# CoderWZW/ARLib

Measured on AMD Instinct MI355X. Metric: BPR-train interactions/sec (LightGCN d=64 L=3 + BPR + Adam, B=2048), higher is better.
Workload: dtype f32

## Files before the change

### arlib_amd/_lib.py

```python
import ctypes as C
import os

_HERE = os.path.dirname(os.path.abspath(__file__))
LIB_PATH = os.environ.get('ARLIB_AMD_LIB') or os.path.join(_HERE, 'lib', 'libarlib_amd.so')
ABI_VERSION = 27
_lib = None


class ArlError(RuntimeError):
    pass


class arl_csr(C.Structure):
    _fields_ = [('n_rows', C.c_int64), ('nnz', C.c_int64), ('rowptr', C.c_void_p), ('col', C.c_void_p), ('val', C.c_void_p),
                ('chunk', C.c_int32), ('n_chunks', C.c_int64), ('chunk_row', C.c_void_p), ('chunk_begin', C.c_void_p),
                ('chunk_end', C.c_void_p), ('n_long', C.c_int64), ('long_row', C.c_void_p), ('long_first', C.c_void_p),
                ('long_count', C.c_void_p), ('partial', C.c_void_p), ('row_tasks', C.c_void_p)]


class arl_blocked(C.Structure):
    _fields_ = [('n_waves', C.c_int64), ('rows_per_wave', C.c_int64), ('loads_in_flight', C.c_int64), ('wave_ptr', C.c_void_p), ('wave_rows', C.c_void_p), ('rec_col', C.c_void_p),
                ('rec_val', C.c_void_p), ('n_split', C.c_int64), ('split_row', C.c_void_p), ('split_first', C.c_void_p), ('split_count', C.c_void_p),
                ('partial', C.c_void_p), ('waves_per_group', C.c_int64)]


class arl_tiled(C.Structure):
    _fields_ = [('n_sweeps', C.c_int64), ('n_slots', C.c_int64), ('cap', C.c_int64), ('n_cb', C.c_int64), ('nnz', C.c_int64),
                ('n_groups', C.c_int64), ('bin_rows', C.c_void_p), ('seg_ptr', C.c_void_p), ('e_col', C.c_void_p), ('e_val', C.c_void_p),
                ('e_row', C.c_void_p)]


_vp, _i64, _i32, _f = C.c_void_p, C.c_int64, C.c_int32, C.c_float
_SIGS = {
    'arl_abi_version': (C.c_int, []),
    'arl_mt_seed': (C.c_int, [_vp, _vp, _i64]),
    'arl_sampler_shuffle': (C.c_int, [_vp, _vp, _i64]),
    'arl_mt_sample_range': (C.c_int, [_vp, _i64, _i64, C.c_int32, _vp, _vp]),
    'arl_sampler_next_batch': (C.c_int, [_vp, _vp, _i64, _i64, _i32, _vp, _vp, _i64, _vp, _vp, _vp]),
    'arl_norm_adj_values_f32': (C.c_int, [_i64, _vp, _vp, _vp, _vp, _vp, _vp]),
    'arl_norm_adj_values_coo_f32': (C.c_int, [_i64, _vp, _vp, _vp, _vp, _i64, _vp, _vp, _vp]),
    'arl_norm_vals_coo_f32': (C.c_int, [_vp, _vp, _vp, _i64, _vp, _vp, _vp]),
    'arl_spmm_csr_f32': (C.c_int, [C.POINTER(arl_csr), _vp, _i64, _f, _f, _vp, _vp, _vp]),
    'arl_spmm_csr_layersum_f32': (C.c_int, [C.POINTER(arl_csr), _vp, _i64, _vp, _vp, _vp, _vp]),
    'arl_spmm_csr_adam_f32': (C.c_int, [C.POINTER(arl_csr), _vp, _i64, _f, _f, _vp, _vp, _vp, _vp, _vp, _f, _f, _f, _f, _i64, _vp]),
    'arl_spmm_blocked_f32': (C.c_int, [C.POINTER(arl_blocked), _vp, _i64, _f, _f, _vp, _vp, _vp, _vp]),
    'arl_spmm_csr_rscale_f32': (C.c_int, [C.POINTER(arl_csr), _vp, _i64, _vp, _f, _f, _vp, _vp, _vp]),
    'arl_spmm_blocked_rscale_f32': (C.c_int, [C.POINTER(arl_blocked), _vp, _i64, _vp, _f, _f, _vp, _vp, _vp]),
    'arl_spmm_blocked_layersum_f32': (C.c_int, [C.POINTER(arl_blocked), _vp, _i64, _vp, _vp, _vp, _vp]),
    'arl_spmm_blocked_adam_f32': (C.c_int, [C.POINTER(arl_blocked), _vp, _i64, _f, _f, _vp, _vp, _vp, _vp, _vp, _f, _f, _f, _f, _i64, _vp]),
    'arl_lpt_deal': (C.c_int, [_i64, _vp, _i64, _i64, _vp, _vp]),
    'arl_syn_v1_pairs': (_i64, [_i64, _i64, C.c_double, C.c_uint64, C.c_double, _i64, _i64, _vp, _i64]),
    'arl_graph_digest': (C.c_uint64, [_vp, _i64]),
    'arl_spmm_tiled_f32': (C.c_int, [C.POINTER(arl_tiled), _vp, _i64, _f, _f, _vp, _vp, _vp, _vp]),
    'arl_spmm_tiled_adam_f32': (C.c_int, [C.POINTER(arl_tiled), _vp, _i64, _f, _f, _vp, _vp, _vp, _vp, _vp, _f, _f, _f, _f, _i64, _vp]),
    'arl_spmm_csr_flagged_f32': (C.c_int, [C.POINTER(arl_csr), _vp, _i64, _vp, _f, _f, _vp, _vp, _vp, _vp]),
    'arl_spmm_csr_rows_workspace_bytes': (_i64, [_i64, _i64, _i64]),
    'arl_spmm_csr_rows_f32': (C.c_int, [C.POINTER(arl_csr), _vp, _i64, _vp, _i64, _i64, _vp, _i64, _f, _vp, _vp, _vp, _vp]),
    'arl_mark_rows_u8': (C.c_int, [_vp, _vp, _i64, _i32, _vp]),
    'arl_mark_rows_bits_u32': (C.c_int, [_vp, _vp, _i64, _i32, _vp]),
    'arl_zero_rows_f32': (C.c_int, [_vp, _vp, _i64, _i64, _vp]),
    'arl_batch_rows_set_f32': (C.c_int, [_vp, _vp, _vp, _vp, _i64, _i64, _vp, _f, _vp, _vp, _vp]),
    'arl_batch_rows_clear_f32': (C.c_int, [_vp, _vp, _vp, _vp, _i64, _i64, _vp, _vp]),
    'arl_bpr_l2_workspace_bytes': (_i64, [_i64]),
    'arl_bpr_l2_fwd_bwd_f32': (C.c_int, [_vp, _i64, _i64, _vp, _vp, _vp, _i64, _f, _f, _vp, _vp, _vp, _i32, _vp]),
    'arl_bpr_l2_partial_f32': (C.c_int, [_vp, _i64, _i64, _vp, _vp, _vp, _i64, _i64, _vp, _vp, _vp]),
    'arl_bpr_l2_backward_f32': (C.c_int, [_vp, _i64, _i64, _vp, _vp, _vp, _i64, _f, _f, _vp, _vp, _vp, _vp]),
    'arl_adam_dense_f32': (C.c_int, [_vp, _vp, _vp, _vp, _i64, _f, _f, _f, _f, _i64, _vp]),
    'arl_sgd_dense_f32': (C.c_int, [_vp, _vp, _i64, _f, _vp]),
    'arl_gather_rows_f32': (C.c_int, [_vp, _vp, _i64, _i64, _vp, _vp]),
    'arl_scatter_add_rows_f32': (C.c_int, [_vp, _vp, _i64, _i64, _vp, _f, _vp]),
    'arl_rows_axpy_unique_f32': (C.c_int, [_vp, _vp, _vp, _i64, _i64, _f, _vp, _vp]),
    'arl_shard_batch_prep_i32': (C.c_int, [_vp, _vp, _vp, _i64, _i64, _i64, _vp, _vp, _vp, _vp, _vp]),
    'arl_infonce_workspace_bytes': (_i64, [_i64, _i64]),
    'arl_infonce_fwd_bwd_f32': (C.c_int, [_vp, _vp, _i64, _i64, _f, _f, _vp, _vp, _vp, _vp, _vp]),
    'arl_simgcl_perturb_f32': (C.c_int, [_vp, _vp, _i64, _i64, _f, _vp]),
    'arl_simgcl_perturb_rng_f32': (C.c_int, [_vp, _vp, _i64, _i64, _vp, _f, C.c_uint64, C.c_uint64, _vp]),
    'arl_ngcf_combine_f32': (C.c_int, [_vp, _vp, _i64, _i64, _vp, _vp]),
    'arl_ngcf_act_f32': (C.c_int, [_vp, _vp, _i64, _i64, _f, _vp]),
    'arl_ngcf_act_bwd_f32': (C.c_int, [_vp, _vp, _i64, _i64, _f, _vp, _vp]),
    'arl_ngcf_combine_bwd_f32': (C.c_int, [_vp, _vp, _vp, _i64, _i64, _vp, _vp, _vp]),
    'arl_ngcf_dense_fwd_f32': (C.c_int, [_vp, _vp, _vp, _i64, _i64, _f, _vp, _vp]),
    'arl_ngcf_dense_dgrad_f32': (C.c_int, [_vp, _vp, _vp, _vp, _vp, _i64, _i64, _f, _vp, _vp, _vp, _vp]),
    'arl_ngcf_wgrad_workspace_bytes': (_i64, [_i64, _i64]),
    'arl_ngcf_dense_wgrad_f32': (C.c_int, [_vp, _vp, _vp, _i64, _i64, _vp, _vp, _vp]),
    'arl_ncf_tower_fwd_f32': (C.c_int, [_vp, _vp, _vp, _i64, _i64, _vp, _vp, _vp, _vp, _vp, _vp, _vp, _vp, _vp, _vp]),
    'arl_ncf_tower_bwd_workspace_bytes': (_i64, [_i64, _i64]),
    'arl_ncf_tower_bwd_f32': (C.c_int, [_vp, _vp, _vp, _vp, _vp, _vp, _i64, _i64, _vp, _vp, _vp, _vp, _vp, _vp, _vp]),
    'arl_wrmf_l2_workspace_bytes': (_i64, [_i64]),
# ... 74 lines not shown
```

### arlib_amd/csrc/arl_host.cpp

```cpp
#include <cstdint>
#include <cstddef>
#include <queue>
#include <cmath>
#include <algorithm>
#include <utility>
#include <vector>
#include "arlib_amd.h"

namespace {

class PyMersenne {
public:
    explicit PyMersenne(uint32_t *state) : w_(state), pos_(state[kN]) {}
    ~PyMersenne() { w_[kN] = pos_; }

    uint32_t next32() {
        if (pos_ >= kN) refill();
        uint32_t y = w_[pos_++];
        y ^= y >> 11;
        y ^= (y << 7) & 0x9d2c5680u;
        y ^= (y << 15) & 0xefc60000u;
        return y ^ (y >> 18);
    }

// ... 23 lines not shown
        w[kN] = kN;
    }

private:
    static constexpr uint32_t kN = 624, kM = 397;
    static uint32_t twist(uint32_t hi, uint32_t lo, uint32_t far) {
        const uint32_t y = (hi & 0x80000000u) | (lo & 0x7fffffffu);
        return far ^ (y >> 1) ^ ((y & 1u) ? 0x9908b0dfu : 0u);
    }
    void refill() {
        for (uint32_t k = 0; k < kN - kM; ++k) w_[k] = twist(w_[k], w_[k + 1], w_[k + kM]);
        for (uint32_t k = kN - kM; k < kN - 1; ++k) w_[k] = twist(w_[k], w_[k + 1], w_[k + kM - kN]);
        w_[kN - 1] = twist(w_[kN - 1], w_[0], w_[kM - 1]);
        pos_ = 0;
    }
    uint32_t *w_;
    uint32_t pos_;
};

inline bool user_has_item(const int64_t *rowptr, const int32_t *items, int64_t rows, int32_t user, int32_t item) {
    if (user < 0 || user >= rows) return false;
    const int32_t *lo = items + rowptr[user], *hi = items + rowptr[user + 1];
    while (lo < hi) {
        const int32_t *mid = lo + (hi - lo) / 2;
        if (*mid < item) lo = mid + 1; else hi = mid;
    }
    return lo < items + rowptr[user + 1] && *lo == item;
}

}

extern "C" {

int arl_abi_version(void) { return 27; }

int arl_mt_seed(uint32_t *mt_state, const uint32_t *key, int64_t key_len) {
    if (!mt_state || !key) return ARL_E_NULL;
    if (key_len < 1) return ARL_E_ARG;
    PyMersenne::seed_by_array(mt_state, key, key_len);
    return ARL_OK;
}

int arl_sampler_shuffle(uint32_t *mt_state, int32_t *pairs, int64_t nnz) {
    if (!mt_state || (!pairs && nnz > 0)) return ARL_E_NULL;
    if (nnz < 0 || nnz > 0xFFFFFFFFll) return ARL_E_RANGE;
    if (mt_state[624] > 624) return ARL_E_ARG;
    PyMersenne rng(mt_state);
    int64_t *rows = reinterpret_cast<int64_t *>(pairs);
    const bool aligned = (reinterpret_cast<uintptr_t>(pairs) & 7u) == 0;
    constexpr int kAhead = 512;
    int64_t js[kAhead];
    for (int64_t i = nnz - 1; i >= 1;) {
        const int cnt = (int)(i < kAhead ? i : kAhead);
        for (int t = 0; t < cnt; ++t) {
            js[t] = rng.below((uint32_t)(i - t + 1));
            __builtin_prefetch(pairs + 2 * js[t], 1, 0);
        }
        if (aligned) {
            for (int t = 0; t < cnt; ++t) { const int64_t a = i - t, j = js[t], v = rows[a]; rows[a] = rows[j]; rows[j] = v; }
        } else {
            for (int t = 0; t < cnt; ++t)
                for (int c = 0; c < 2; ++c) { const int64_t a = i - t, j = js[t]; const int32_t v = pairs[2 * a + c]; pairs[2 * a + c] = pairs[2 * j + c]; pairs[2 * j + c] = v; }
        }
        i -= cnt;
    }
    return ARL_OK;
}
// ... 130 lines not shown
```

### arlib_amd/csrc/arl_kernels.hip

```cpp
#include <hip/hip_runtime.h>
#include <stdint.h>
#include <math.h>
#include <stdio.h>
#include <stdlib.h>
#include "arlib_amd.h"
#include <type_traits>

#define ARL_LAUNCH_CHECK()                                  \
    do {                                                    \
        hipError_t e__ = hipGetLastError();                 \
        if (e__ != hipSuccess) return (int)e__;             \
    } while (0)

namespace {

constexpr int kWave = 64;
constexpr int kBlock = 256;
constexpr int kWavesPerBlock = kBlock / kWave;

__device__ __forceinline__ float wave_sum(float v) {
#pragma unroll
    for (int off = 32; off > 0; off >>= 1) v += __shfl_xor(v, off);
    return v;
}
// ... 417 lines not shown
#pragma unroll
                    for (int i = 0; i < 4; ++i) { const int k = k0 + 64 * i + lane; x[q][i] = k < d ? s[k] : 0.f; }
                }
#pragma unroll
                for (int q = 0; q < 4; ++q) {
                    if (tt[q] < 0) continue;
#pragma unroll
                    for (int i = 0; i < 4; ++i) { const float c = sc[q] * x[q][i]; acc[i] = acc[i] + c; }
                }
            }
        });
        if (!owner) return;
#pragma unroll
        for (int i = 0; i < 4; ++i) { const int k = k0 + 64 * i + lane; if (k < d) o[k] = acc[i]; }
    }
    if (MARK && lane == 0) {
        flags[row] = 1;
        atomicOr(bits + (row >> 5), 1u << (row & 31));
    }
}
__global__ __launch_bounds__(kBlock) void batch_rows_clear_kernel(float *__restrict__ G, uint8_t *__restrict__ flags, uint32_t *__restrict__ bits,
                                                                   const int32_t *__restrict__ idx, int n, int d, uint32_t *__restrict__ dup) {
    const int lane = threadIdx.x & 63;
    const int t = blockIdx.x * kWavesPerBlock + (threadIdx.x >> 6);
    if (t >= n) return;
    const int row = idx[t];
    float *o = G + (size_t)row * d;
    for (int k = lane; k < d; k += kWave) o[k] = 0.f;
    if (lane == 0) {
        flags[row] = 0;
        atomicAnd(bits + (row >> 5), ~(1u << (row & 31)));
        if (dup) atomicAnd(dup + (row >> 5), ~(1u << (row & 31)));
    }
}

struct TiledDev {
    int n_sweeps, n_slots, cap, n_cb, n_groups;
    const int32_t *bin_rows;
    const int32_t *seg_ptr;
    const int32_t *e_col;
    const float *e_val;
    const uint16_t *e_row;
};

constexpr int kTiledThreads = 1024;
constexpr int kTiledWaves = kTiledThreads / kWave;

template <int LPR, int MODE>
__global__ __launch_bounds__(kTiledThreads) void spmm_tiled_kernel(TiledDev T, const float *__restrict__ X, int d, Epi ep) {
    constexpr int G = kWave / LPR;
    extern __shared__ float acc_lds[];
    const int ld = d + 4;
    const int tid = threadIdx.x, lane = tid & 63, wv = tid >> 6;
    const int g = lane / LPR, q = lane % LPR;
    const int og = wv * G + g;
    const bool qact = q * 4 < d;
    const float *xq = X + q * 4;
    for (int sweep = 0; sweep < T.n_sweeps; ++sweep) {
        const int bin = sweep * T.n_slots + blockIdx.x;
        for (int t = tid; t < T.cap * ld; t += kTiledThreads) acc_lds[t] = 0.f;
        const int lo = T.seg_ptr[(size_t)bin * T.n_groups + og], hi = T.seg_ptr[(size_t)bin * T.n_groups + og + 1];
        __syncthreads();
        int c_n = 0, r_n = -1;
        float v_n = 0.f;
        if (lo + q < hi) { c_n = T.e_col[lo + q]; v_n = T.e_val[lo + q]; r_n = T.e_row[lo + q]; }
        for (int base = lo; __any(base < hi); base += LPR) {
// ... 3619 lines not shown

int arl_spmm_tiled_f32(const arl_tiled *T, const float *X, int64_t d, float alpha, float beta, const float *Z, const uint8_t *zflags, float *Y,
                       arl_stream_t stream) {
    if (!Y) return ARL_E_NULL;
    if (beta != 0.f && !Z) return ARL_E_NULL;
    if (Y == X) return ARL_E_ARG;
    Epi ep = {};
    ep.alpha = alpha; ep.beta = beta; ep.Z = (beta != 0.f) ? Z : nullptr; ep.zflags = zflags; ep.Y = Y;
    return launch_spmm_tiled<EPI_AXPBY>(T, X, d, ep, (hipStream_t)stream);
}

int arl_spmm_tiled_adam_f32(const arl_tiled *T, const float *X, int64_t d, float alpha, float beta, const float *Z, const uint8_t *zflags,
                            float *P, float *M, float *V, float lr, float beta1, float beta2, float eps, int64_t step, arl_stream_t stream) {
    if (!P || !M || !V) return ARL_E_NULL;
    if (beta != 0.f && !Z) return ARL_E_NULL;
    if (step < 1 || P == X) return ARL_E_ARG;
    Epi ep = {};
    ep.alpha = alpha; ep.beta = beta; ep.Z = (beta != 0.f) ? Z : nullptr; ep.zflags = zflags; ep.P = P; ep.M = M; ep.V = V;
    {
        const AdamScalars a = adam_scalars(lr, beta1, beta2, step);
        ep.step_size = a.step_size; ep.bc2_sqrt = a.bc2_sqrt; ep.w1 = a.w1; ep.b2 = a.b2; ep.w2 = a.w2; ep.eps = (float)typed_double(eps);
    }
    return launch_spmm_tiled<EPI_ADAM>(T, X, d, ep, (hipStream_t)stream);
}

int arl_spmm_csr_flagged_f32(const arl_csr *A, const float *X, int64_t d, const uint32_t *xbits, float alpha, float beta, const float *Z,
                             const uint8_t *zflags, float *Y, arl_stream_t stream) {
    if (!Y) return ARL_E_NULL;
    if (beta != 0.f && !Z) return ARL_E_NULL;
    if (Y == X) return ARL_E_ARG;
    Epi ep = {};
    ep.alpha = alpha; ep.beta = beta; ep.Z = (beta != 0.f) ? Z : nullptr; ep.zflags = zflags; ep.Y = Y;
    return launch_spmm<EPI_AXPBY>(A, X, d, ep, (hipStream_t)stream, xbits);
}

int arl_spmm_csr_adam_f32(const arl_csr *A, const float *X, int64_t d, float alpha, float beta, const float *Z, const uint8_t *zflags, float *P,
                          float *M, float *V, float lr, float beta1, float beta2, float eps, int64_t step, arl_stream_t stream) {
    if (!P || !M || !V) return ARL_E_NULL;
    if (beta != 0.f && !Z) return ARL_E_NULL;
    if (step < 1) return ARL_E_ARG;
    if (P == X) return ARL_E_ARG;
    Epi ep = {};
    ep.alpha = alpha; ep.beta = beta; ep.Z = (beta != 0.f) ? Z : nullptr; ep.zflags = zflags; ep.P = P; ep.M = M; ep.V = V;
    {
        const AdamScalars a = adam_scalars(lr, beta1, beta2, step);
        ep.step_size = a.step_size; ep.bc2_sqrt = a.bc2_sqrt; ep.w1 = a.w1; ep.b2 = a.b2; ep.w2 = a.w2; ep.eps = (float)typed_double(eps);
    }
    return launch_spmm<EPI_ADAM>(A, X, d, ep, (hipStream_t)stream);
}

int64_t arl_spmm_csr_rows_workspace_bytes(int64_t n_rows_sel, int64_t nsplit, int64_t d) {
    return (n_rows_sel < 0 || nsplit < 1 || d < 0) ? 0 : (int64_t)sizeof(float) * n_rows_sel * nsplit * d;
}

int arl_spmm_csr_rows_f32(const arl_csr *A, const float *X, int64_t d, const int32_t *rows, int64_t n_rows_sel, int64_t nsplit,
                          const float *const *layers, int64_t n_layers, float alpha, const float *row_weight, float *out_c, void *workspace,
                          arl_stream_t stream) {
    if (!A || !X || !rows || !out_c || !workspace || !A->rowptr) return ARL_E_NULL;
    if (A->nnz > 0 && (!A->col || !A->val)) return ARL_E_NULL;
    if (n_layers < 0 || n_layers > 8 || (n_layers > 0 && !layers)) return ARL_E_ARG;
    if (d <= 0 || d > 256 || (d & 3)) return ARL_E_DIM;
    if (n_rows_sel < 0 || nsplit < 1 || nsplit > 1024 || n_rows_sel * nsplit > 0x7fffffffll) return ARL_E_RANGE;
    if (n_rows_sel == 0) return ARL_OK;
    hipStream_t st = (hipStream_t)stream;
    CsrDev D = {};
    D.n_rows = (int)A->n_rows; D.rowptr = A->rowptr; D.col = A->col; D.val = A->val;
// ... 1086 lines not shown
```

### arlib_amd/engine.py

```python
import torch

from . import ops


def mean_adjacency_gradient(A, E0, G, L, s, out, noises=None, eps=0.1):
    if L == 0:
        return out
    E = [E0]
    for k in range(L - 1):
        nxt = ops.spmm(A, E[-1])
        if noises is not None:
            ops.simgcl_perturb_(nxt, noises[k], eps)
        E.append(nxt)
    G = G.contiguous()
    acc = G
    for j in range(L):
        ops.sddmm_csr(A, acc, E[L - 1 - j], s, out=out)
        if j < L - 1:
            acc = ops.spmm(A, acc, 1.0, 1.0, G)
    return out


class PropagationEngine:
    def __init__(self, graph, n_users, n_items, emb_size, n_layers, reg, lr, device, skip_layer0=False,
# ... 6 lines not shown
        self.optimizer = optimizer
        self.device = torch.device(device)
        if self.device.type != 'cuda':
            raise ops._lib.ArlError('PropagationEngine needs a GPU device (no CPU fallback)')
        if graph is None and self.L > 0:
            raise ValueError('n_layers > 0 needs a graph')
        if graph is not None and graph.n_rows != self.N:
            raise ValueError('graph has %d rows, expected U+I=%d' % (graph.n_rows, self.N))
        if self.L > 0:
            ops._check_width(self.d, 'PropagationEngine')
        if self.skip0 and self.L < 1:
            raise ValueError('skip_layer0 needs n_layers >= 1')
        if schedule not in ('auto', 'csr', 'blocked'):
            raise ValueError("schedule must be 'auto', 'csr' or 'blocked'")
        if schedule != 'csr':
            ops.auto_blocked(graph, emb_size, split=self.U, force=(schedule == 'blocked'))
        if graph is not None and graph.nnz >= ops.BLOCKED_MIN_NNZ:
            graph.enable_masked_order()
        z = lambda: torch.zeros(self.N, self.d, dtype=torch.float32, device=self.device)
        self.E0 = z() if table is None else table
        if self.E0.shape != (self.N, self.d) or self.E0.dtype != torch.float32 or not self.E0.is_contiguous():
            raise ValueError('table must be contiguous fp32 [U+I, d]')
        self.m, self.v, self.G = z(), z(), z()
        if self.L > 0:
            self.S, self.Ea, self.Eb = z(), z(), z()
        else:
            self.S = self.E0
        self.t = 0
        self.loss_out = torch.zeros(4, dtype=torch.float32, device=self.device)
        self._G_dirty = True
        self._noise_seed, self._noise_stream = None, 0
        self.nsplit = 32
        self.flags = self.bits = self.dup_bits = self.hops = None
        self._sparse_B, self._sb_cache = None, {}
        self.Gc = self.out_c = self.rows_ws = self.ar = self.arB = self._ws = None
        self._sgl_acc = self._sgl_hops = None
        self.ngcf_W = self.ngcf_m = self.ngcf_v = None

    @property
    def user_emb(self):
        return self.E0[:self.U]

    @property
    def item_emb(self):
        return self.E0[self.U:]

    def forward(self, noises=None, eps=0.1, out=None):
        L, A = self.L, self.A
        if L == 0:
            return self.E0
        S = self.S if out is None else out
        if noises is None and not self.skip0:
            if L == 1:
                return ops.spmm(A, self.E0, 0.5, 0.5, self.E0, out=S)
            ops.spmm_layersum(A, self.E0, self.E0, S, self.Ea)
            cur, nxt = self.Ea, self.Eb
            for _ in range(L - 2):
                ops.spmm_layersum(A, cur, S, S, nxt)
                cur, nxt = nxt, cur
            s = 1.0 / (L + 1)
            return ops.spmm(A, cur, s, s, S, out=S)
        cur, nxt, x = self.Ea, self.Eb, self.E0
        for k in range(L):
            ops.spmm(A, x, out=cur)
            if noises is not None:
                ops.simgcl_perturb_(cur, noises[k], eps)
# ... 51 lines not shown
    def _begin_sparse(self, B):
        self._sparse_buffers(B)
        if self._G_dirty:
            self.G.zero_()
            self._G_dirty = False

    def _batch_rows(self, u, p, n):
        return torch.cat([u, p + self.U, n + self.U])

    def _contrast_rows(self, u, p):
        uidx = torch.unique(u.long())
        iidx = torch.unique(p.long()) + self.U
        return torch.cat([uidx, iidx]).to(torch.int32), uidx.numel()

    def _streams(self, n):
        if self._noise_seed is None:
            self._noise_seed = int(torch.randint(0, 2 ** 62, (1,)).item())
            self._noise_stream = 0
        first = self._noise_stream
        self._noise_stream += n
        return self._noise_seed, first

    def _mean_rows(self, graph, hops, rows, out=None, workspace=None):
        layers = [self.E0]
        for k in range(self.L - 1):
            layers.append(ops.spmm(graph, layers[-1], out=hops[k]))
        return ops.spmm_rows(graph, layers[-1], rows, layers, 1.0 / (self.L + 1), nsplit=self.nsplit, out=out, workspace=workspace, check_range=False)

    def _bpr_compact(self, out_c, B):
        self.Gc.zero_()
        ops.bpr_l2_fwd_bwd(out_c, B, self.ar, self.ar, self.arB, self.reg, self.Gc, workspace=self._ws, loss_out=self.loss_out, check_range=False, distinct_rows=True)

    def _set_rows(self, rows, grad):
        ops.batch_rows_set_(self.G, self.flags, self.bits, rows, grad, 1.0, check_range=False, dup_bits=self.dup_bits)

    def _mark_rows(self, rows):
        ops.mark_rows_(self.flags, rows, 1, check_range=False)
        ops.mark_bits_(self.bits, rows, True, self.N, check_range=False)

    def _clear_rows(self, rows):
        ops.batch_rows_clear_(self.G, self.flags, self.bits, rows, check_range=False, dup_bits=self.dup_bits)

    def _masked_hops(self, graph, bufs, src=None, after_hop=None):
        acc, bits = self.G if src is None else src, self.bits
        for k in range(self.L - 1):
            acc = ops.spmm_flagged(graph, acc, bits, 1.0, 1.0, self.G, self.flags, out=bufs[k % len(bufs)])
            bits = None
            if after_hop is not None:
                after_hop(self.L - 1 - k, acc)
        return acc, bits

    def loss_and_grad_out(self, out, u, p, n):
        self.G.zero_()
        self._G_dirty = True
        if self._ws is None or self._ws.numel() < 4 * u.numel():
            self._ws = torch.empty(4 * u.numel(), dtype=torch.float32, device=self.device)
        ops.bpr_l2_fwd_bwd(out, self.U, u, p, n, self.reg, self.G, workspace=self._ws, loss_out=self.loss_out, check_range=False)
        return self.loss_out

    def grad(self, u, p, n):
        out = self.forward()
        lo = self.loss_and_grad_out(out, u, p, n)
        return lo, self.backward_to_table(self.G)

    def step(self, u, p, n, rows=None):
        if self.optimizer != 'adam' or self.L == 0 or self.skip0 or self.L > 8:
            return self.step_dense(u, p, n)
        return self._step_sparse(u, p, n, rows, None)

    def _step_sparse(self, u, p, n, rows, extra_grad):
        L, A = self.L, self.A
        B = u.numel()
        if rows is None:
            rows = self._batch_rows(u, p, n)
        self._begin_sparse(B)
        s = 1.0 / (L + 1)
        self._mean_rows(A, self.hops, rows, out=self.out_c, workspace=self.rows_ws)
        self._bpr_compact(self.out_c, B)
        if extra_grad is not None:
# ... 231 lines not shown

        def backward_into(graph, sel, grad_c, accumulate):
            self._set_rows(sel, grad_c)
            acc, bits = self._masked_hops(graph, self._sgl_hops)
            tmp = ops.spmm_flagged(graph, acc, bits, s, s, self.G, self.flags, out=self._sgl_hops[0] if L == 1 else self.hops[0])
            if accumulate:
                self._sgl_acc.add_(tmp)
            else:
                self._sgl_acc.copy_(tmp)
            self._clear_rows(sel)

        out_c = self._mean_rows(self.A, self._sgl_hops, rows)
        self._bpr_compact(out_c, B)
        v1 = self._mean_rows(view1, self._sgl_hops, rows_cl)
        v2 = self._mean_rows(view2, self._sgl_hops, rows_cl)
        lcl, d1, d2 = ops.infonce_fwd_bwd(v1, v2, tau)
        cl_loss = cl_rate * lcl[0]
        backward_into(self.A, rows, self.Gc, False)
        backward_into(view1, rows_cl, d1 * cl_rate, True)
        backward_into(view2, rows_cl, d2 * cl_rate, True)
        self.t += 1
        ops.adam_dense(self.E0, self._sgl_acc, self.m, self.v, self.lr, self.t, self.betas, self.eps)
        return self.loss_out, cl_loss

    def _sparse_buffers(self, B):
        if self._sparse_B == B:
            return
        dev, d = self.device, self.d
        if self.flags is None:
            self.flags = torch.zeros(self.N, dtype=torch.uint8, device=dev)
            self.bits = torch.zeros((self.N + 31) // 32, dtype=torch.int32, device=dev)
            self.dup_bits = torch.zeros_like(self.bits)
            self.hops = [self.Ea, self.Eb] + [torch.empty_like(self.Ea) for _ in range(max(0, self.L - 3))]
        sb = self._sb_cache.get(B)
        if sb is None:
            ar = torch.arange(B, dtype=torch.int32, device=dev)
            sb = (torch.zeros(3 * B, d, dtype=torch.float32, device=dev), torch.empty(3 * B, d, dtype=torch.float32, device=dev),
                  torch.empty(3 * B * self.nsplit * d, dtype=torch.float32, device=dev), ar, ar + B, torch.empty(4 * B, dtype=torch.float32, device=dev))
            if len(self._sb_cache) >= 8:
                del self._sb_cache[next(iter(self._sb_cache))]
            self._sb_cache[B] = sb
        self.Gc, self.out_c, self.rows_ws, self.ar, self.arB, self._ws = sb
        self._sparse_B = B

    def step_dense(self, u, p, n):
        L, A = self.L, self.A
        out = self.forward()
        lo = self.loss_and_grad_out(out, u, p, n)
        self.t += 1
        if self.optimizer == 'adam' and L > 0 and not self.skip0:
            acc, _ = self._dense_hops(self.G)
            s = 1.0 / (L + 1)
            ops.spmm_adam(A, acc, s, s, self.G, self.E0, self.m, self.v, self.lr, self.t, self.betas, self.eps)
            return lo
        g = self.backward_to_table(self.G)
        self.apply_grad(g)
        return lo

    def apply_grad(self, g):
        if self.optimizer == 'adam':
            ops.adam_dense(self.E0, g, self.m, self.v, self.lr, self.t, self.betas, self.eps)
        elif self.optimizer == 'sgd':
            ops.sgd_dense(self.E0, g, self.lr)
        else:
            raise ValueError('unknown optimizer %r' % (self.optimizer,))

# ... 4 lines not shown
```

### arlib_amd/ops.py

```python
import ctypes as C
import os
import time
import numpy as np
import torch

from . import _lib
from ._lib import arl_csr, check

DEFAULT_CHUNK = 512
EVENT_HOOK = None


_raw_stream = getattr(torch._C, '_cuda_getCurrentRawStream', None)


def _stream():
    if _raw_stream is not None:
        return C.c_void_p(_raw_stream(torch.cuda.current_device()))
    return C.c_void_p(torch.cuda.current_stream().cuda_stream)


def _dev(t, dtype, name, ndim=None):
    if not isinstance(t, torch.Tensor):
        raise TypeError('%s: expected a torch.Tensor' % name)
# ... 598 lines not shown
    _spmm_dispatch(A, d, lambda p: check(L.arl_spmm_blocked_adam_f32(p, _ptr(X), d, alpha, beta, zp, _ptr(zflags), _ptr(P), _ptr(M), _ptr(V), lr, betas[0],
                                                                     betas[1], eps, int(step), st), 'arl_spmm_blocked_adam_f32'),
                   lambda p: check(L.arl_spmm_csr_adam_f32(p, _ptr(X), d, alpha, beta, zp, _ptr(zflags), _ptr(P), _ptr(M), _ptr(V), lr, betas[0], betas[1], eps,
                                                           int(step), st), 'arl_spmm_csr_adam_f32'))
    if tok is not None:
        EVENT_HOOK.end(tok)


def spmm_flagged(A, X, xflags=None, alpha=1.0, beta=0.0, Z=None, zflags=None, out=None):
    d = _check_xy(A, X, 'X', A.n_cols)
    Y = torch.empty(A.n_rows, d, dtype=torch.float32, device=X.device) if out is None else out
    if _check_xy(A, Y, 'out') != d or Y.data_ptr() == X.data_ptr():
        raise ValueError('spmm_flagged: out must be [n_rows, d] and must not alias X')
    if beta != 0.0 and (Z is None or _check_xy(A, Z, 'Z') != d):
        raise ValueError('spmm_flagged: Z [n_rows, d] required when beta != 0')
    if xflags is not None:
        _dev(xflags, torch.int32, 'xflags (bitmap)', 1)
        if xflags.numel() != (A.n_cols + 31) // 32:
            raise ValueError('spmm_flagged: bitmap needs ceil(n_cols/32) int32 words')
    if zflags is not None:
        _check_flags(zflags, A.n_rows, 'zflags')
    L, zp, st = _lib.lib(), (_ptr(Z) if beta != 0.0 else None), _stream()
    tok = EVENT_HOOK.begin('masked' if xflags is not None else 'axpby') if EVENT_HOOK is not None else None
    csr = lambda p: check(L.arl_spmm_csr_flagged_f32(p, _ptr(X), d, _ptr(xflags), alpha, beta, zp, _ptr(zflags), _ptr(Y), st), 'arl_spmm_csr_flagged_f32')
    if xflags is not None:
        csr(C.byref(A._struct(d)))
    else:
        _spmm_dispatch(A, d, lambda p: check(L.arl_spmm_blocked_f32(p, _ptr(X), d, alpha, beta, zp, _ptr(zflags), _ptr(Y), st), 'arl_spmm_blocked_f32'), csr)
    if tok is not None:
        EVENT_HOOK.end(tok)
    return Y


ROWS_NSPLIT = 16


def spmm_rows(A, X, rows, layers=(), alpha=1.0, nsplit=ROWS_NSPLIT, out=None, workspace=None, check_range=True, row_weight=None):
    d = _check_xy(A, X, 'X', A.n_cols)
    _dev(rows, torch.int32, 'rows', 1)
    n = rows.numel()
    if check_range and n and (int(rows.min()) < 0 or int(rows.max()) >= A.n_rows):
        raise IndexError('spmm_rows: row index out of range')
    if len(layers) > 8:
        raise ValueError('spmm_rows: at most 8 layer tables')
    for t in layers:
        if _check_xy(A, t, 'layer') != d:
            raise ValueError('spmm_rows: layer table shape mismatch')
    if out is None:
        out = torch.empty(n, d, dtype=torch.float32, device=X.device)
    _dev(out, torch.float32, 'out', 2)
    if out.shape != (n, d):
        raise ValueError('spmm_rows: out must be [len(rows), d]')
    need = _lib.lib().arl_spmm_csr_rows_workspace_bytes(n, nsplit, d) // 4
    if workspace is None or workspace.numel() < need:
        workspace = torch.empty(max(need, 1), dtype=torch.float32, device=X.device)
    arr = (C.c_void_p * max(len(layers), 1))(*[t.data_ptr() for t in layers])
    s = A._struct(d)
    tok = EVENT_HOOK.begin('rows') if EVENT_HOOK is not None else None
    if row_weight is not None and (_dev(row_weight, torch.float32, 'row_weight', 1).numel() != n):
        raise ValueError('spmm_rows: row_weight must have one entry per listed row')
    check(_lib.lib().arl_spmm_csr_rows_f32(C.byref(s), _ptr(X), d, _ptr(rows), n, nsplit, C.cast(arr, C.c_void_p), len(layers), alpha, _ptr(row_weight),
                                           _ptr(out), _ptr(workspace), _stream()), 'arl_spmm_csr_rows_f32')
    if tok is not None:
        EVENT_HOOK.end(tok)
    return out

# ... 1151 lines not shown
```

### include/arlib_amd.h

```cpp
#ifndef ARLIB_AMD_H
#define ARLIB_AMD_H

#include <stdint.h>

#ifdef __cplusplus
extern "C" {
#endif

#define ARL_OK 0
#define ARL_E_NULL (-1)
#define ARL_E_DIM (-2)
#define ARL_E_RANGE (-3)
#define ARL_E_ARG (-4)

typedef void *arl_stream_t;

int arl_abi_version(void);

int arl_mt_seed(uint32_t *mt_state, const uint32_t *key, int64_t key_len);
int arl_sampler_shuffle(uint32_t *mt_state, int32_t *pairs, int64_t nnz);
int arl_mt_sample_range(uint32_t *mt_state, int64_t n, int64_t k, int32_t use_pool, int32_t *out, int32_t *scratch);
int arl_sampler_next_batch(uint32_t *mt_state, const int32_t *pairs, int64_t begin, int64_t count,
                           int32_t n_items, const int64_t *memb_rowptr, const int32_t *memb_items,
                           int64_t memb_rows, int32_t *out_u, int32_t *out_p, int32_t *out_n);
// ... 4 lines not shown
    const int32_t *rowptr;
    const int32_t *col;
    const float *val;
    int32_t chunk;
    int64_t n_chunks;
    const int32_t *chunk_row;
    const int32_t *chunk_begin;
    const int32_t *chunk_end;
    int64_t n_long;
    const int32_t *long_row;
    const int32_t *long_first;
    const int32_t *long_count;
    float *partial;
    const int32_t *row_tasks;
} arl_csr;

int arl_norm_adj_values_f32(int64_t n_rows, const int32_t *rowptr, const int32_t *col, const float *w,
                            float *dinv, float *val, arl_stream_t stream);
int arl_norm_adj_values_coo_f32(int64_t n_rows, const int32_t *rowptr, const int32_t *erow, const int32_t *col,
                                const float *w, int64_t nnz, float *dinv, float *val, arl_stream_t stream);
int arl_norm_vals_coo_f32(const int32_t *erow, const int32_t *col, const float *w, int64_t nnz, const float *dinv, float *val,
                          arl_stream_t stream);

int arl_spmm_csr_f32(const arl_csr *A, const float *X, int64_t d, float alpha, float beta, const float *Z,
                     float *Y, arl_stream_t stream);
int arl_spmm_csr_layersum_f32(const arl_csr *A, const float *X, int64_t d, const float *S_in, float *S,
                              float *Y, arl_stream_t stream);
int arl_spmm_csr_adam_f32(const arl_csr *A, const float *X, int64_t d, float alpha, float beta, const float *Z,
                          const uint8_t *zflags, float *P, float *M, float *V, float lr, float beta1, float beta2,
                          float eps, int64_t step, arl_stream_t stream);

int arl_spmm_csr_flagged_f32(const arl_csr *A, const float *X, int64_t d, const uint32_t *xbits, float alpha, float beta,
                             const float *Z, const uint8_t *zflags, float *Y, arl_stream_t stream);
int64_t arl_spmm_csr_rows_workspace_bytes(int64_t n_rows_sel, int64_t nsplit, int64_t d);
int arl_spmm_csr_rows_f32(const arl_csr *A, const float *X, int64_t d, const int32_t *rows, int64_t n_rows_sel,
                          int64_t nsplit, const float *const *layers, int64_t n_layers, float alpha, const float *row_weight,
                          float *out_c, void *workspace, arl_stream_t stream);
int arl_mark_rows_u8(uint8_t *flags, const int32_t *idx, int64_t n, int32_t value, arl_stream_t stream);
int arl_mark_rows_bits_u32(uint32_t *bits, const int32_t *idx, int64_t n, int32_t set, arl_stream_t stream);
int arl_zero_rows_f32(float *dst, const int32_t *idx, int64_t n, int64_t d, arl_stream_t stream);
int arl_batch_rows_set_f32(float *G, uint8_t *flags, uint32_t *bits, const int32_t *idx, int64_t n, int64_t d,
                           const float *src, float scale, const float *row_scale, uint32_t *dup_bits, arl_stream_t stream);
int arl_batch_rows_clear_f32(float *G, uint8_t *flags, uint32_t *bits, const int32_t *idx, int64_t n, int64_t d,
                             uint32_t *dup_bits, arl_stream_t stream);

typedef struct arl_blocked {
    int64_t n_waves, rows_per_wave;
    int64_t loads_in_flight;
    const int32_t *wave_ptr;
    const int32_t *wave_rows;
    const int32_t *rec_col;
    const float *rec_val;
    int64_t n_split;
    const int32_t *split_row;
    const int32_t *split_first;
    const int32_t *split_count;
    float *partial;
    int64_t waves_per_group;
} arl_blocked;
int arl_spmm_blocked_f32(const arl_blocked *P, const float *X, int64_t d, float alpha, float beta, const float *Z,
                         const uint8_t *zflags, float *Y, arl_stream_t stream);
int arl_spmm_csr_rscale_f32(const arl_csr *A, const float *X, int64_t d, const float *row_scale, float alpha, float beta,
                            const float *Z, float *Y, arl_stream_t stream);
int arl_spmm_blocked_rscale_f32(const arl_blocked *P, const float *X, int64_t d, const float *row_scale, float alpha,
                                float beta, const float *Z, float *Y, arl_stream_t stream);
int arl_spmm_blocked_layersum_f32(const arl_blocked *P, const float *X, int64_t d, const float *S_in, float *S, float *Y,
// ... 166 lines not shown
```

Measured before the change: 320,000.

## Add push-based sparse SpMM for first masked backward hop over batch rows

Adds a push-style SpMM for the first masked hop of the backward pass. Batch rows are claimed, their neighbour lists are scattered as (source, weight) records into per-destination slots, and each destination row then sorts its records and sums them in a fixed order. Only edges touching the sparse gradient rows are visited, instead of a pull over the full CSR with flag checks. It is enabled only for graphs with at least 6M nonzeros. It adds atomics, per-row sorting work and a scratch buffer the size of nnz, and it launches a collect kernel over all rows.

```diff
diff --git a/arlib_amd/_lib.py b/arlib_amd/_lib.py
--- a/arlib_amd/_lib.py
+++ b/arlib_amd/_lib.py
@@ -3,7 +3,7 @@
 
 _HERE = os.path.dirname(os.path.abspath(__file__))
 LIB_PATH = os.environ.get('ARLIB_AMD_LIB') or os.path.join(_HERE, 'lib', 'libarlib_amd.so')
-ABI_VERSION = 27
+ABI_VERSION = 28
 _lib = None
 
 
@@ -54,6 +54,8 @@
     'arl_spmm_tiled_f32': (C.c_int, [C.POINTER(arl_tiled), _vp, _i64, _f, _f, _vp, _vp, _vp, _vp]),
     'arl_spmm_tiled_adam_f32': (C.c_int, [C.POINTER(arl_tiled), _vp, _i64, _f, _f, _vp, _vp, _vp, _vp, _vp, _f, _f, _f, _f, _i64, _vp]),
     'arl_spmm_csr_flagged_f32': (C.c_int, [C.POINTER(arl_csr), _vp, _i64, _vp, _f, _f, _vp, _vp, _vp, _vp]),
+    'arl_spmm_batch_push_sort_cap': (_i64, [_i64]),
+    'arl_spmm_batch_push_f32': (C.c_int, [C.POINTER(arl_csr), _vp, _i64, _vp, _i64, _f, _f, _vp, _vp, _vp, _vp, _vp, _vp]),
     'arl_spmm_csr_rows_workspace_bytes': (_i64, [_i64, _i64, _i64]),
     'arl_spmm_csr_rows_f32': (C.c_int, [C.POINTER(arl_csr), _vp, _i64, _vp, _i64, _i64, _vp, _i64, _f, _vp, _vp, _vp, _vp]),
     'arl_mark_rows_u8': (C.c_int, [_vp, _vp, _i64, _i32, _vp]),
diff --git a/arlib_amd/csrc/arl_host.cpp b/arlib_amd/csrc/arl_host.cpp
--- a/arlib_amd/csrc/arl_host.cpp
+++ b/arlib_amd/csrc/arl_host.cpp
@@ -79,7 +79,7 @@
 
 extern "C" {
 
-int arl_abi_version(void) { return 27; }
+int arl_abi_version(void) { return 28; }
 
 int arl_mt_seed(uint32_t *mt_state, const uint32_t *key, int64_t key_len) {
     if (!mt_state || !key) return ARL_E_NULL;
diff --git a/arlib_amd/csrc/arl_kernels.hip b/arlib_amd/csrc/arl_kernels.hip
--- a/arlib_amd/csrc/arl_kernels.hip
+++ b/arlib_amd/csrc/arl_kernels.hip
@@ -473,6 +473,199 @@
         atomicAnd(bits + (row >> 5), ~(1u << (row & 31)));
         if (dup) atomicAnd(dup + (row >> 5), ~(1u << (row & 31)));
     }
+}
+
+constexpr int kPushSplit = 32;
+constexpr int kPushPiece = 4 * kWave;
+constexpr int kPushLdsCap = 512;
+constexpr unsigned long long kPushNone = ~0ull;
+
+__global__ __launch_bounds__(kBlock) void push_claim_kernel(uint32_t *__restrict__ claim, const int32_t *__restrict__ rows, int n, int n_rows,
+                                                             uint8_t *__restrict__ owner) {
+    const int t = blockIdx.x * kBlock + threadIdx.x;
+    if (t >= n) return;
+    const int r = rows[t];
+    uint8_t own = 0;
+    if ((unsigned)r < (unsigned)n_rows) {
+        const uint32_t m = 1u << (r & 31);
+        own = (atomicOr(claim + (r >> 5), m) & m) ? 0 : 1;
+    }
+    owner[t] = own;
+}
+
+__global__ __launch_bounds__(kBlock) void push_scatter_kernel(CsrDev A, const int32_t *__restrict__ rows, const uint8_t *__restrict__ owner, int n,
+                                                               int32_t *__restrict__ cnt, int2 *__restrict__ rec) {
+    const int lane = threadIdx.x & (kWave - 1);
+    const long long task = (long long)blockIdx.x * kWavesPerBlock + (threadIdx.x >> 6);
+    if (task >= (long long)n * kPushSplit) return;
+    const int t = (int)(task / kPushSplit), s = (int)(task % kPushSplit);
+    if (!owner[t]) return;
+    const int r = rows[t];
+    const long long end = A.rowptr[r + 1];
+    for (long long base = (long long)A.rowptr[r] + (long long)s * kPushPiece; base < end; base += (long long)kPushSplit * kPushPiece) {
+        int c[4], k[4], b[4], w[4];
+        float v[4];
+        bool ok[4];
+#pragma unroll
+        for (int u = 0; u < 4; ++u) {
+            const long long e = base + u * kWave + lane;
+            ok[u] = e < end;
+            c[u] = 0; v[u] = 0.f;
+            if (ok[u]) { c[u] = A.col[e]; v[u] = A.val[e]; }
+            ok[u] = ok[u] && (unsigned)c[u] < (unsigned)A.n_rows;
+        }
+#pragma unroll
+        for (int u = 0; u < 4; ++u) {
+            k[u] = 0; b[u] = 0; w[u] = 0;
+            if (ok[u]) { b[u] = A.rowptr[c[u]]; w[u] = A.rowptr[c[u] + 1] - b[u]; k[u] = atomicAdd(cnt + c[u], 1); }
+        }
+#pragma unroll
+        for (int u = 0; u < 4; ++u)
+            if (ok[u] && k[u] < w[u]) rec[(size_t)b[u] + k[u]] = make_int2(r, __float_as_int(v[u]));
+    }
+}
+
+__device__ __forceinline__ unsigned long long push_key(int2 x, int n_rows) {
+    const uint32_t r = min((uint32_t)x.x, (uint32_t)(n_rows - 1));
+    return ((unsigned long long)r << 32) | (uint32_t)x.y;
+}
+
+template <int LPR>
+__device__ __forceinline__ float4 push_sum_sorted(const int2 *__restrict__ rec, int c, int n_rows, const float *__restrict__ gq, int d, bool qact, int g, int q) {
+    unsigned long long key = kPushNone;
+    if (q < c) { const int2 x = rec[q]; key = push_key(x, n_rows); }
+    float4 acc = make_float4(0.f, 0.f, 0.f, 0.f);
+    for (;;) {
+        unsigned long long gm = key;
+#pragma unroll
+        for (int off = 1; off < LPR; off <<= 1) { const unsigned long long o = __shfl_xor(gm, off); gm = o < gm ? o : gm; }
+        if (!__any(gm != kPushNone)) break;
+        const unsigned long long bal = __ballot(gm != kPushNone && key == gm);
+        const unsigned long long mine = (bal >> (g * LPR)) & ((LPR == 64) ? ~0ull : ((1ull << (LPR & 63)) - 1ull));
+        if (mine && q == __ffsll((long long)mine) - 1) key = kPushNone;
+        if (gm != kPushNone && qact) fma4(acc, __uint_as_float((uint32_t)gm), *reinterpret_cast<const float4 *>(gq + (size_t)(uint32_t)(gm >> 32) * d));
+    }
+    return acc;
+}
+
+template <int LPR>
+__device__ __forceinline__ float4 push_sum_wave(const int2 *__restrict__ rec, int c, int n_rows, unsigned long long *keys, const float *__restrict__ gq, int d, bool qact,
+                                                int lane) {
+    constexpr int R = kPushLdsCap / kWave;
+    unsigned long long own[R];
+    int rank[R];
+#pragma unroll
+    for (int k = 0; k < R; ++k) {
+        const int i = lane + k * kWave;
+        own[k] = kPushNone; rank[k] = 0;
+        if (i < c) { const int2 x = rec[i]; own[k] = push_key(x, n_rows); keys[i] = own[k]; }
+    }
+    __builtin_amdgcn_wave_barrier();
+    for (int j = 0; j < c; ++j) {
+        const unsigned long long kj = keys[j];
+#pragma unroll
+        for (int k = 0; k < R; ++k) rank[k] += (kj < own[k] || (kj == own[k] && j < lane + k * kWave)) ? 1 : 0;
+    }
+    __builtin_amdgcn_wave_barrier();
+#pragma unroll
+    for (int k = 0; k < R; ++k)
+        if (lane + k * kWave < c) keys[rank[k]] = own[k];
+    __builtin_amdgcn_wave_barrier();
+    float4 acc = make_float4(0.f, 0.f, 0.f, 0.f);
+    for (int p0 = 0; p0 < c; p0 += 8) {
+        unsigned long long kk[8];
+        float4 x[8];
+#pragma unroll
+        for (int u = 0; u < 8; ++u) kk[u] = keys[min(p0 + u, c - 1)];
+#pragma unroll
+        for (int u = 0; u < 8; ++u) {
+            x[u] = make_float4(0.f, 0.f, 0.f, 0.f);
+            if (qact && p0 + u < c) x[u] = *reinterpret_cast<const float4 *>(gq + (size_t)(uint32_t)(kk[u] >> 32) * d);
+        }
+#pragma unroll
+        for (int u = 0; u < 8; ++u)
+            if (p0 + u < c) fma4(acc, __uint_as_float((uint32_t)kk[u]), x[u]);
+    }
+    __builtin_amdgcn_wave_barrier();
+    return acc;
+}
+
+template <int LPR>
+__device__ __forceinline__ float4 push_sum_scan(const int2 *__restrict__ rec, int c, int n_rows, const float *__restrict__ gq, int d, bool qact, int q) {
+    constexpr int kNoSlot = 0x7fffffff;
+    float4 acc = make_float4(0.f, 0.f, 0.f, 0.f);
+    unsigned long long last = 0ull;
+    int last_slot = -1;
+    for (;;) {
+        unsigned long long bk = kPushNone;
+        int bs = kNoSlot;
+        for (int i = q; i < c; i += LPR) {
+            const int2 x = rec[i];
+            const unsigned long long key = push_key(x, n_rows);
+            const bool after = key > last || (key == last && i > last_slot);
+            if (after && (key < bk || (key == bk && i < bs))) { bk = key; bs = i; }
+        }
+#pragma unroll
+        for (int off = 1; off < LPR; off <<= 1) {
+            const unsigned long long ok = __shfl_xor(bk, off);
+            const int os = __shfl_xor(bs, off);
+            if (ok < bk || (ok == bk && os < bs)) { bk = ok; bs = os; }
+        }
+        if (!__any(bs != kNoSlot)) break;
+        if (bs != kNoSlot) {
+            if (qact) fma4(acc, __uint_as_float((uint32_t)bk), *reinterpret_cast<const float4 *>(gq + (size_t)(uint32_t)(bk >> 32) * d));
+            last = bk; last_slot = bs;
+        }
+    }
+    return acc;
+}
+
+template <int LPR>
+__global__ __launch_bounds__(kBlock) void push_collect_kernel(CsrDev A, const float *__restrict__ G, int d, float alpha, float beta, float *__restrict__ Y,
+                                                               int32_t *__restrict__ cnt, uint32_t *__restrict__ claim, const int2 *__restrict__ rec) {
+    constexpr int GR = kWave / LPR;
+    const int lane = threadIdx.x & (kWave - 1);
+    const int g = lane / LPR, q = lane % LPR;
+    const long long task = ((long long)blockIdx.x * kWavesPerBlock + (threadIdx.x >> 6)) * GR + g;
+    const int row = task < A.n_rows ? (int)(A.n_rows - 1 - task) : -1;
+    int c = 0, b = 0;
+    bool listed = false;
+    if (row >= 0) {
+        c = cnt[row];
+        listed = (claim[row >> 5] >> (row & 31)) & 1u;
+    }
+    if (c > 0) {
+        b = A.rowptr[row];
+        if (q == 0) cnt[row] = 0;
+        c = min(c, A.rowptr[row + 1] - b);
+    }
+    if (listed && q == 0) atomicAnd(claim + (row >> 5), ~(1u << (row & 31)));
+    const bool qact = (q * 4 < d);
+    const float *gq = G + q * 4;
+    float4 acc = make_float4(0.f, 0.f, 0.f, 0.f);
+    if (__any(c > 0)) acc = push_sum_sorted<LPR>(rec + b, c <= LPR ? c : 0, A.n_rows, gq, d, qact, g, q);
+    if (__any(c > LPR)) {
+        __shared__ unsigned long long lds_keys[kWavesPerBlock][kPushLdsCap];
+#pragma unroll 1
+        for (int gi = 0; gi < GR; ++gi) {
+            const int cg = __shfl(c, gi * LPR), bg = __shfl(b, gi * LPR);
+            if (cg <= LPR || cg > kPushLdsCap) continue;
+            const float4 a = push_sum_wave<LPR>(rec + bg, cg, A.n_rows, lds_keys[threadIdx.x >> 6], gq, d, qact, lane);
+            if (g == gi) acc = a;
+        }
+        if (__any(c > kPushLdsCap)) {
+            const float4 a = push_sum_scan<LPR>(rec + b, c > kPushLdsCap ? c : 0, A.n_rows, gq, d, qact, q);
+            if (c > kPushLdsCap) acc = a;
+        }
+    }
+    if (row < 0 || !qact) return;
+    const size_t o = (size_t)row * d + q * 4;
+    float4 y = make_float4(alpha * acc.x, alpha * acc.y, alpha * acc.z, alpha * acc.w);
+    if (listed && beta != 0.f) {
+        const float4 z = *reinterpret_cast<const float4 *>(G + o);
+        y.x = fmaf(beta, z.x, y.x); y.y = fmaf(beta, z.y, y.y); y.z = fmaf(beta, z.z, y.z); y.w = fmaf(beta, z.w, y.w);
+    }
+    *reinterpret_cast<float4 *>(Y + o) = y;
 }
 
 struct TiledDev {
@@ -4158,6 +4351,41 @@
     Epi ep = {};
     ep.alpha = alpha; ep.beta = beta; ep.Z = (beta != 0.f) ? Z : nullptr; ep.zflags = zflags; ep.Y = Y;
     return launch_spmm<EPI_AXPBY>(A, X, d, ep, (hipStream_t)stream, xbits);
+}
+
+int64_t arl_spmm_batch_push_sort_cap(int64_t d) { return (d <= 0) ? 0 : kPushLdsCap; }
+
+int arl_spmm_batch_push_f32(const arl_csr *A, const float *G, int64_t d, const int32_t *rows, int64_t n, float alpha, float beta, int32_t *cnt,
+                            uint32_t *claim, uint8_t *owner, void *rec, float *Y, arl_stream_t stream) {
+    if (!A || !G || !Y || !cnt || !claim || (A->n_rows > 0 && !A->rowptr) || (A->nnz > 0 && (!A->col || !A->val || !rec))) return ARL_E_NULL;
+    if (n > 0 && (!rows || !owner)) return ARL_E_NULL;
+    if (d <= 0 || d > 256 || (d & 3)) return ARL_E_DIM;
+    if (A->n_rows < 0 || A->n_rows > 0x7fffffffll || A->nnz > 0x7fffffffll || n < 0 || n * kPushSplit > 0x7fffffffll) return ARL_E_RANGE;
+    if (Y == G || ((uintptr_t)rec & 7)) return ARL_E_ARG;
+    if (A->n_rows == 0) return ARL_OK;
+    hipStream_t st = (hipStream_t)stream;
+    CsrDev D = {};
+    D.n_rows = (int)A->n_rows; D.rowptr = A->rowptr; D.col = A->col; D.val = A->val;
+    const int di = (int)d, ni = (int)n;
+    int2 *r2 = (int2 *)rec;
+    if (ni > 0) {
+        hipLaunchKernelGGL(push_claim_kernel, dim3((unsigned)((ni + kBlock - 1) / kBlock)), dim3(kBlock), 0, st, claim, rows, ni, D.n_rows, owner);
+        ARL_LAUNCH_CHECK();
+        const long long tasks = (long long)ni * kPushSplit;
+        hipLaunchKernelGGL(push_scatter_kernel, dim3((unsigned)((tasks + kWavesPerBlock - 1) / kWavesPerBlock)), dim3(kBlock), 0, st, D, rows, (const uint8_t *)owner, ni, cnt, r2);
+        ARL_LAUNCH_CHECK();
+    }
+#define ARL_PUSH_CASE(LPRV)                                                                                                    \
+    hipLaunchKernelGGL((push_collect_kernel<LPRV>), dim3((unsigned)((D.n_rows + kWavesPerBlock * (kWave / LPRV) - 1) / (kWavesPerBlock * (kWave / LPRV)))), \
+                       dim3(kBlock), 0, st, D, G, di, alpha, beta, Y, cnt, claim, (const int2 *)r2)
+    if (d <= 16) ARL_PUSH_CASE(4);
+    else if (d <= 32) ARL_PUSH_CASE(8);
+    else if (d <= 64) ARL_PUSH_CASE(16);
+    else if (d <= 128) ARL_PUSH_CASE(32);
+    else ARL_PUSH_CASE(64);
+#undef ARL_PUSH_CASE
+    ARL_LAUNCH_CHECK();
+    return ARL_OK;
 }
 
 int arl_spmm_csr_adam_f32(const arl_csr *A, const float *X, int64_t d, float alpha, float beta, const float *Z, const uint8_t *zflags, float *P,
diff --git a/arlib_amd/engine.py b/arlib_amd/engine.py
--- a/arlib_amd/engine.py
+++ b/arlib_amd/engine.py
@@ -62,6 +62,8 @@
         self._noise_seed, self._noise_stream = None, 0
         self.nsplit = 32
         self.flags = self.bits = self.dup_bits = self.hops = None
+        self.push = None
+        self._rows = None
         self._sparse_B, self._sb_cache = None, {}
         self.Gc = self.out_c = self.rows_ws = self.ar = self.arB = self._ws = None
         self._sgl_acc = self._sgl_hops = None
@@ -179,19 +181,25 @@
         ops.bpr_l2_fwd_bwd(out_c, B, self.ar, self.ar, self.arB, self.reg, self.Gc, workspace=self._ws, loss_out=self.loss_out, check_range=False, distinct_rows=True)
 
     def _set_rows(self, rows, grad):
+        self._rows = rows
         ops.batch_rows_set_(self.G, self.flags, self.bits, rows, grad, 1.0, check_range=False, dup_bits=self.dup_bits)
 
     def _mark_rows(self, rows):
+        self._rows = rows
         ops.mark_rows_(self.flags, rows, 1, check_range=False)
         ops.mark_bits_(self.bits, rows, True, self.N, check_range=False)
 
     def _clear_rows(self, rows):
+        self._rows = None
         ops.batch_rows_clear_(self.G, self.flags, self.bits, rows, check_range=False, dup_bits=self.dup_bits)
 
     def _masked_hops(self, graph, bufs, src=None, after_hop=None):
         acc, bits = self.G if src is None else src, self.bits
         for k in range(self.L - 1):
-            acc = ops.spmm_flagged(graph, acc, bits, 1.0, 1.0, self.G, self.flags, out=bufs[k % len(bufs)])
+            if k == 0 and acc is self.G and self.push is not None and self._rows is not None and graph.n_rows == self.N and graph.nnz <= self.push.nnz:
+                acc = ops.spmm_batch_push(graph, self.G, self._rows, 1.0, 1.0, self.push, out=bufs[0], check_range=False)
+            else:
+                acc = ops.spmm_flagged(graph, acc, bits, 1.0, 1.0, self.G, self.flags, out=bufs[k % len(bufs)])
             bits = None
             if after_hop is not None:
                 after_hop(self.L - 1 - k, acc)
@@ -489,6 +497,8 @@
             self.bits = torch.zeros((self.N + 31) // 32, dtype=torch.int32, device=dev)
             self.dup_bits = torch.zeros_like(self.bits)
             self.hops = [self.Ea, self.Eb] + [torch.empty_like(self.Ea) for _ in range(max(0, self.L - 3))]
+            if self.L >= 2 and self.A.nnz >= ops.PUSH_MIN_NNZ:
+                self.push = ops.BatchPushScratch(self.N, self.A.nnz, dev)
         sb = self._sb_cache.get(B)
         if sb is None:
             ar = torch.arange(B, dtype=torch.int32, device=dev)
diff --git a/arlib_amd/ops.py b/arlib_amd/ops.py
--- a/arlib_amd/ops.py
+++ b/arlib_amd/ops.py
@@ -654,6 +654,52 @@
     return Y
 
 
+PUSH_MIN_NNZ = 6_000_000
+
+
+class BatchPushScratch:
+
+    def __init__(self, n_rows, nnz, device):
+        self.n_rows, self.nnz = int(n_rows), int(nnz)
+        self.cnt = torch.zeros(self.n_rows, dtype=torch.int32, device=device)
+        self.claim = torch.zeros((self.n_rows + 31) // 32, dtype=torch.int32, device=device)
+        self.rec = torch.empty(max(self.nnz, 1), dtype=torch.int64, device=device)
+        self._owner = None
+
+    def owner(self, n):
+        if self._owner is None or self._owner.numel() < n:
+            self._owner = torch.empty(max(n, 1), dtype=torch.uint8, device=self.cnt.device)
+        return self._owner
+
+
+def batch_push_sort_cap(d):
+    return int(_lib.lib().arl_spmm_batch_push_sort_cap(int(d)))
+
+
+def spmm_batch_push(A, G, rows, alpha=1.0, beta=0.0, scratch=None, out=None, check_range=True):
+    d = _check_xy(A, G, 'G', A.n_cols)
+    if A.n_rows != A.n_cols:
+        raise ValueError('spmm_batch_push: A must be square (and symmetric)')
+    _dev(rows, torch.int32, 'rows', 1)
+    n = rows.numel()
+    if check_range and n and (int(rows.min()) < 0 or int(rows.max()) >= A.n_rows):
+        raise IndexError('spmm_batch_push: row index out of range')
+    Y = torch.empty(A.n_rows, d, dtype=torch.float32, device=G.device) if out is None else out
+    if _check_xy(A, Y, 'out') != d or Y.data_ptr() == G.data_ptr():
+        raise ValueError('spmm_batch_push: out must be [n_rows, d] and must not alias G')
+    if scratch is None:
+        scratch = BatchPushScratch(A.n_rows, A.nnz, G.device)
+    if scratch.n_rows != A.n_rows or scratch.nnz < A.nnz:
+        raise ValueError('spmm_batch_push: scratch too small for this graph')
+    s = A._struct(d)
+    tok = EVENT_HOOK.begin('masked') if EVENT_HOOK is not None else None
+    check(_lib.lib().arl_spmm_batch_push_f32(C.byref(s), _ptr(G), d, _ptr(rows), n, alpha, beta, _ptr(scratch.cnt), _ptr(scratch.claim),
+                                             _ptr(scratch.owner(n)), _ptr(scratch.rec), _ptr(Y), _stream()), 'arl_spmm_batch_push_f32')
+    if tok is not None:
+        EVENT_HOOK.end(tok)
+    return Y
+
+
 ROWS_NSPLIT = 16
 
 
diff --git a/include/arlib_amd.h b/include/arlib_amd.h
--- a/include/arlib_amd.h
+++ b/include/arlib_amd.h
@@ -60,6 +60,9 @@
 
 int arl_spmm_csr_flagged_f32(const arl_csr *A, const float *X, int64_t d, const uint32_t *xbits, float alpha, float beta,
                              const float *Z, const uint8_t *zflags, float *Y, arl_stream_t stream);
+int64_t arl_spmm_batch_push_sort_cap(int64_t d);
+int arl_spmm_batch_push_f32(const arl_csr *A, const float *G, int64_t d, const int32_t *rows, int64_t n, float alpha, float beta,
+                            int32_t *cnt, uint32_t *claim, uint8_t *owner, void *rec, float *Y, arl_stream_t stream);
 int64_t arl_spmm_csr_rows_workspace_bytes(int64_t n_rows_sel, int64_t nsplit, int64_t d);
 int arl_spmm_csr_rows_f32(const arl_csr *A, const float *X, int64_t d, const int32_t *rows, int64_t n_rows_sel,
                           int64_t nsplit, const float *const *layers, int64_t n_layers, float alpha, const float *row_weight,
```

Result: slower. 306,200 (-4.3%).
